# iebeid/ProtGram-DirectGCN

Hardware: AMD Instinct MI355X
Metric: edges/sec propagated, DirectGCN fwd on 4-gram graph, 1/2/4/8 MI355X (higher is better)
Workload: dtype f32; 1 GPU; directgcn_fwd_B(20,4); graph=complete n-gram de Bruijn B(20,4), num_nodes=160000, transitions=3200000, nnz_per_adjacency=6559580, feat_dim=128, layers=2, classes=20, propagation=precomputed-weights, entry=trainer COO (edge_index_*/edge_weight_* -> csr_from_coo), parallelism=single

## Files before the change

### include/pg_directgcn.h

```cpp
#ifndef PG_DIRECTGCN_H
#define PG_DIRECTGCN_H

#include <stdint.h>

#ifdef __cplusplus
extern "C" {
#endif

#define PG_ABI_VERSION 4

#define PG_OK 0
#define PG_ERR_ARG (-1)
#define PG_ERR_HIP (-2)
#define PG_ERR_UNSUPPORTED (-3)

typedef struct pg_edge3 {
    int32_t col;
    float w_in;
    float w_out;
    float w_und;
} pg_edge3_t;

typedef struct pg_edgeraw {
    int32_t col;
    float a_fwd;
    float a_bwd;
    float m_und;
} pg_edgeraw_t;

typedef struct pg_edge1 {
    int32_t col;
    float w;
} pg_edge1_t;


#define PG_FLAG_NO_XCD_REMAP (1u << 0)
#define PG_FLAG_EDGE_LDS (1u << 1)
#define PG_FLAG_UNROLL4 (1u << 2)
#define PG_FLAG_BCAST_RECORDS (1u << 7)
#define PG_FLAG_NGRAMT_WIDE (1u << 8)
#define PG_FLAG_NGRAMT_HALVES (1u << 4)
#define PG_FLAG_NGRAMT_NARROW (1u << 3)
#define PG_FLAG_DENSE_PREGATED (1u << 14)
#define PG_FLAG_DENSE_TILED (1u << 15)
#define PG_FLAG_DENSE_X3 (1u << 16)
#define PG_FLAG_WGRAD_BF16_TILED (1u << 11)
#define PG_FLAG_DGRAD_BF16_TILED (1u << 10)
#define PG_FLAG_DGRAD_BF16_RESIDENT (1u << 9)
#define PG_FLAG_WGRAD_F32MFMA (1u << 18)
#define PG_FLAG_DGRAD_F32MFMA (1u << 17)
#define PG_FLAG_NO_NGRAM (1u << 20)
#define PG_FLAG_NGRAM_BLOCK4 (1u << 21)
#define PG_FLAG_MID_NO_PAIRS (1u << 22)
#define PG_FLAG_MID_LOADER_SYNC (1u << 19)
#define PG_FLAG_DENSE_NO_IL (1u << 13)
#define PG_FLAG_DENSE_A_CACHED (1u << 12)
#define PG_FLAG_SCATTER_CPW_SHIFT 24
#define PG_FLAG_MID_TRANSPOSED (1u << 23)


const char* pg_last_error(void);
int pg_abi_version(void);

int pg_spmm3_f32(int64_t n_rows, const int64_t* rowptr, const int32_t* row_order, const pg_edge3_t* edges,
                 const float* X, int64_t ldx, int64_t F,
                 float* Z, int64_t ldz, uint32_t flags, void* stream);


int pg_spmm3_fusednorm_f32(int64_t n_rows, const int64_t* rowptr, const int32_t* row_order,
                           const pg_edgeraw_t* edges,
                           const float* node_norm, float eps,
                           const float* X, int64_t ldx, int64_t F,
                           float* Z, int64_t ldz, uint32_t flags, void* stream);

int pg_edges_normalize_f32(int64_t n_rows, const int64_t* rowptr, const pg_edgeraw_t* raw,
                           const float* node_norm, float eps, pg_edge3_t* out, void* stream);

int pg_spmm3t_f32(int64_t n_rows, const int64_t* rowptr, const int32_t* row_order, const pg_edge3_t* edges,
                  const float* G, int64_t ldg, int64_t F,
                  float* dX, int64_t lddx, int accumulate, uint32_t flags, void* stream);

int pg_spmm1_f32(int64_t n_rows, const int64_t* rowptr, const int32_t* row_order, const pg_edge1_t* edges,
                 const float* X, int64_t ldx, int64_t F,
                 float* Y, int64_t ldy, int accumulate, uint32_t flags, void* stream);

#define PG_GATES_VECTOR 0
#define PG_GATES_SCALAR 1

typedef struct pg_layer_args {
    int64_t M, F_in, F_out;
    const float* Z; int64_t ldz;
    const float* W_main_in; const float* W_main_out; const float* W_undirected; const float* W_shared;
    const float* b_main_in; const float* b_dir_shared_in;
    const float* b_main_out; const float* b_dir_shared_out;
    const float* b_undirected; const float* b_undirected_shared;
    int32_t gate_mode;
    const float* C_in; const float* C_out; const float* C_directed; const float* C_undirected; const float* C_all;
    const int64_t* rows;
    const float* constant; int64_t ld_const;
    const float* res_x; int64_t ld_res;
    const float* W_res; const float* b_res;
    int32_t act; float slope;
    float* Y; int64_t ldy;
    float drop_p; const int64_t* drop_seed;
} pg_layer_args_t;

int64_t pg_directgcn_packed_floats(int64_t F_in, int64_t F_out, int has_res_proj);

int pg_directgcn_pack_f32(const pg_layer_args_t* args, float* packed, void* stream);

int pg_directgcn_dense_f32(const pg_layer_args_t* args, const float* packed, uint32_t flags, void* stream);

int pg_directgcn_dense_ngram_rows_f32(const pg_layer_args_t* args, const float* packed, int64_t Kn1, int64_t m0,
                                      int32_t map_res, int32_t map_y, uint32_t flags, void* stream);

int pg_spmm3_gated_f32(int64_t n_rows, const int64_t* rowptr, const int32_t* row_order, const pg_edge3_t* edges,
                       const float* X, int64_t ldx, int64_t F, const pg_layer_args_t* gates,
                       float* Z, int64_t ldz, uint32_t flags, void* stream);

int64_t pg_ngram_plan_floats(int K, int n, int64_t n_rows);
int pg_ngram_plan_f32(int K, int n, int64_t n_rows, const int64_t* rowptr, const pg_edge3_t* edges, float* plan,
                      int64_t plan_floats, int* bad, void* stream);
int pg_spmm3_ngram_f32(int K, int n, int64_t n_rows, const float* plan, const float* X, int64_t ldx, int64_t F,
                       const pg_layer_args_t* gates, float* Z, int64_t ldz, uint32_t flags, void* stream);
int pg_spmm3t_ngram_f32(int K, int n, int64_t n_rows, const float* plan, const float* G, int64_t ldg, int64_t F,
                        float* dX, int64_t lddx, int accumulate, uint32_t flags, void* stream);
int pg_spmm3t_ngram_bf16(int K, int n, int64_t n_rows, const float* plan, const uint16_t* G, int64_t ldg, int64_t F,
                         uint16_t* dX, int64_t lddx, int accumulate, uint32_t flags, void* stream);
int pg_spmm3t_ngram_add_bf16(int K, int n, int64_t n_rows, const float* plan, const uint16_t* G, int64_t ldg,
                             int64_t F, const uint16_t* C, int64_t ldc, uint16_t* dX, int64_t lddx, uint32_t flags,
                             void* stream);

int64_t pg_ngram_mplan_floats(int K, int n, int64_t n_rows);
int pg_ngram_mplan_f32(int K, int n, int64_t n_rows, const int64_t* rowptr, const pg_edge3_t* edges, float* plan,
                       int64_t plan_floats, int* bad, void* stream);
int pg_spmm3_ngram_mid_f32(int K, int n, int64_t n_rows, const float* plan, const float* X, int64_t ldx, int64_t F,
                           const pg_layer_args_t* gates, float* Z, int64_t ldz, uint32_t flags, void* stream);
int pg_spmm3_ngram_mid_rows_f32(int K, int n, int64_t n_rows, const float* plan, const float* X, int64_t ldx, int64_t F,
                                int64_t m_begin, int64_t m_end, float* Z, int64_t ldz, uint32_t flags, void* stream);
// ... 144 lines not shown
```

### protgram-directgcn_amd/_lib.py

```python
from __future__ import annotations

import ctypes
import os

_HERE = os.path.dirname(os.path.abspath(__file__))
_LIB_PATH = os.environ.get("PG_DIRECTGCN_LIB", os.path.join(_HERE, "libpgdgcn.so"))

PG_OK = 0
PG_FLAG_NO_XCD_REMAP = 1 << 0
PG_FLAG_EDGE_LDS = 1 << 1
PG_FLAG_UNROLL4 = 1 << 2
PG_FLAG_BCAST_RECORDS = 1 << 7
PG_FLAG_NGRAMT_WIDE = 1 << 8
PG_FLAG_NGRAMT_NARROW = 1 << 3
PG_FLAG_NGRAMT_HALVES = 1 << 4
PG_FLAG_DENSE_PREGATED = 1 << 14
PG_FLAG_DENSE_TILED = 1 << 15
PG_FLAG_DENSE_X3 = 1 << 16
PG_FLAG_WGRAD_F32MFMA = 1 << 18
PG_FLAG_WGRAD_BF16_TILED = 1 << 11
PG_FLAG_DGRAD_BF16_TILED = 1 << 10
PG_FLAG_DGRAD_BF16_RESIDENT = 1 << 9
PG_FLAG_DGRAD_F32MFMA = 1 << 17
PG_FLAG_NO_NGRAM = 1 << 20
PG_FLAG_NGRAM_BLOCK4 = 1 << 21
PG_FLAG_MID_NO_PAIRS = 1 << 22
PG_FLAG_MID_LOADER_SYNC = 1 << 19
PG_FLAG_MID_TRANSPOSED = 1 << 23
PG_FLAG_SCATTER_CPW_SHIFT = 24
PG_FLAG_DENSE_A_CACHED = 1 << 12
PG_FLAG_DENSE_NO_IL = 1 << 13

c_i64, c_i32, c_u32, c_f32, c_vp = ctypes.c_int64, ctypes.c_int32, ctypes.c_uint32, ctypes.c_float, ctypes.c_void_p


PG_OK, PG_ERR_ARG, PG_ERR_HIP, PG_ERR_UNSUPPORTED = 0, -1, -2, -3


class NativeLibraryError(RuntimeError):
    pass


class LayerArgs(ctypes.Structure):
    _fields_ = [("M", c_i64), ("F_in", c_i64), ("F_out", c_i64),
                ("Z", c_vp), ("ldz", c_i64),
                ("W_main_in", c_vp), ("W_main_out", c_vp), ("W_undirected", c_vp), ("W_shared", c_vp),
                ("b_main_in", c_vp), ("b_dir_shared_in", c_vp),
                ("b_main_out", c_vp), ("b_dir_shared_out", c_vp),
                ("b_undirected", c_vp), ("b_undirected_shared", c_vp),
                ("gate_mode", c_i32),
                ("C_in", c_vp), ("C_out", c_vp), ("C_directed", c_vp), ("C_undirected", c_vp), ("C_all", c_vp),
                ("rows", c_vp),
                ("constant", c_vp), ("ld_const", c_i64),
                ("res_x", c_vp), ("ld_res", c_i64),
                ("W_res", c_vp), ("b_res", c_vp),
                ("act", c_i32), ("slope", c_f32),
                ("Y", c_vp), ("ldy", c_i64),
                ("drop_p", c_f32), ("drop_seed", c_vp)]


class LayerGradArgs(ctypes.Structure):
    _fields_ = [("dY", c_vp), ("lddy", c_i64), ("dpre", c_vp), ("ldp", c_i64), ("dZ", c_vp), ("lddz", c_i64),
                ("dres", c_vp), ("lddres", c_i64), ("dgate", c_vp), ("gates", c_vp), ("dW", c_vp),
                ("work", c_vp), ("work_floats", c_i64), ("dpre_f32", c_vp), ("ldp_f32", c_i64)]


SIGNATURES = {
    "pg_last_error": (ctypes.c_char_p, []),
    "pg_abi_version": (ctypes.c_int, []),
    "pg_spmm3_f32": (ctypes.c_int, [c_i64, c_vp, c_vp, c_vp, c_vp, c_i64, c_i64, c_vp, c_i64, c_u32, c_vp]),
    "pg_spmm3_gated_f32": (ctypes.c_int, [c_i64, c_vp, c_vp, c_vp, c_vp, c_i64, c_i64, ctypes.POINTER(LayerArgs), c_vp,
                                          c_i64, c_u32, c_vp]),
    "pg_spmm3_fusednorm_f32": (ctypes.c_int, [c_i64, c_vp, c_vp, c_vp, c_vp, c_f32, c_vp, c_i64, c_i64, c_vp, c_i64,
                                              c_u32, c_vp]),
    "pg_edges_normalize_f32": (ctypes.c_int, [c_i64, c_vp, c_vp, c_vp, c_f32, c_vp, c_vp]),
    "pg_ngram_plan_floats": (c_i64, [ctypes.c_int, ctypes.c_int, c_i64]),
    "pg_ngram_plan_f32": (ctypes.c_int, [ctypes.c_int, ctypes.c_int, c_i64, c_vp, c_vp, c_vp, c_i64, c_vp, c_vp]),
    "pg_spmm3_ngram_f32": (ctypes.c_int, [ctypes.c_int, ctypes.c_int, c_i64, c_vp, c_vp, c_i64, c_i64,
                                          ctypes.POINTER(LayerArgs), c_vp, c_i64, c_u32, c_vp]),
    "pg_ngram_mplan_floats": (c_i64, [ctypes.c_int, ctypes.c_int, c_i64]),
    "pg_ngram_mplan_f32": (ctypes.c_int, [ctypes.c_int, ctypes.c_int, c_i64, c_vp, c_vp, c_vp, c_i64, c_vp, c_vp]),
    "pg_spmm3_ngram_mid_f32": (ctypes.c_int, [ctypes.c_int, ctypes.c_int, c_i64, c_vp, c_vp, c_i64, c_i64,
                                              ctypes.POINTER(LayerArgs), c_vp, c_i64, c_u32, c_vp]),
    "pg_spmm3_ngram_mid_rows_f32": (ctypes.c_int, [ctypes.c_int, ctypes.c_int, c_i64, c_vp, c_vp, c_i64, c_i64, c_i64,
                                                   c_i64, c_vp, c_i64, c_u32, c_vp]),
    "pg_spmm3_ngram_mid_bf16": (ctypes.c_int, [ctypes.c_int, ctypes.c_int, c_i64, c_vp, c_vp, c_i64, c_i64, c_vp,
                                               c_i64, c_u32, c_vp]),
    "pg_spmm3_ngram_mid_rows_bf16": (ctypes.c_int, [ctypes.c_int, ctypes.c_int, c_i64, c_vp, c_vp, c_i64, c_i64, c_i64,
                                                    c_i64, c_vp, c_i64, c_u32, c_vp]),
    "pg_ngram_mplan_map_f32": (ctypes.c_int, [ctypes.c_int, ctypes.c_int, c_i64, c_vp, c_vp, c_vp, c_vp, c_i64, c_vp,
                                              c_vp]),
    "pg_spmm3_ngram_mid_map_f32": (ctypes.c_int, [ctypes.c_int, ctypes.c_int, c_vp, c_vp, c_vp, c_i64, c_i64, c_vp,
                                                  c_i64, c_u32, c_vp]),
    "pg_spmm3_resid_f32": (ctypes.c_int, [c_i64, c_vp, c_vp, c_vp, c_vp, c_i64, c_i64, c_vp, c_i64, c_u32, c_vp]),
    "pg_rows_gather": (ctypes.c_int, [c_vp, c_i64, c_vp, c_i64, c_i64, c_vp, c_i64, c_vp]),
    "pg_rows_scatter": (ctypes.c_int, [c_vp, c_i64, c_vp, c_i64, c_i64, c_vp, c_i64, c_vp]),
    "pg_rows_gather_sum": (ctypes.c_int, [c_vp, c_i64, c_vp, c_i64, ctypes.c_int, c_vp, c_vp, c_i64, c_i64, c_vp,
                                          c_i64, ctypes.c_int, c_vp]),
    "pg_ngram_scatter_plan": (ctypes.c_int, [ctypes.c_int, ctypes.c_int, c_vp, c_i64, c_i64, c_vp, c_vp]),
    "pg_spmm3t_ngram_scatter_f32": (ctypes.c_int, [c_vp, c_i64, c_vp, c_i64, c_i64, c_vp, c_i64, c_u32, c_vp]),
    "pg_spmm3t_ngram_scatter_bf16": (ctypes.c_int, [c_vp, c_i64, c_vp, c_i64, c_i64, c_vp, c_i64, c_u32, c_vp]),
    "pg_spmm3t_ngram_f32": (ctypes.c_int, [ctypes.c_int, ctypes.c_int, c_i64, c_vp, c_vp, c_i64, c_i64, c_vp, c_i64,
                                           ctypes.c_int, c_u32, c_vp]),
    "pg_spmm3t_ngram_mid_offdiag_f32": (ctypes.c_int, [ctypes.c_int, ctypes.c_int, c_i64, c_vp, c_vp, c_i64, c_i64,
                                                       c_vp, c_i64, ctypes.c_int, c_u32, c_vp]),
    "pg_spmm3t_ngram_mid_bf16": (ctypes.c_int, [ctypes.c_int, ctypes.c_int, c_i64, c_vp, c_vp, c_i64, c_i64, c_vp, c_i64,
                                                ctypes.c_int, c_u32, c_vp]),
    "pg_spmm3t_ngram_bf16": (ctypes.c_int, [ctypes.c_int, ctypes.c_int, c_i64, c_vp, c_vp, c_i64, c_i64, c_vp, c_i64,
                                            ctypes.c_int, c_u32, c_vp]),
    "pg_spmm3t_ngram_add_bf16": (ctypes.c_int, [ctypes.c_int, ctypes.c_int, c_i64, c_vp, c_vp, c_i64, c_i64, c_vp,
                                                c_i64, c_vp, c_i64, c_u32, c_vp]),
    "pg_spmm3t_f32": (ctypes.c_int, [c_i64, c_vp, c_vp, c_vp, c_vp, c_i64, c_i64, c_vp, c_i64, ctypes.c_int, c_u32,
                                     c_vp]),
    "pg_spmm1_f32": (ctypes.c_int, [c_i64, c_vp, c_vp, c_vp, c_vp, c_i64, c_i64, c_vp, c_i64, ctypes.c_int, c_u32,
# ... 82 lines not shown
```

### protgram-directgcn_amd/csrc/pg_dense.hip

```cpp
#include "pg_common.h"
#include "pg_split3.h"

namespace {

typedef float f32x16 __attribute__((ext_vector_type(16)));
typedef float f32x4 __attribute__((ext_vector_type(4)));

constexpr int BK = 32;
constexpr int LDSW = 36;

struct DenseP {
    int64_t M;
    int F_in, F_out, K;
    const float* Z;
    int64_t ldz;
    const float* Bp;
    const float* bsum;
    int gate_mode;
    const float *C_in, *C_out, *C_dir, *C_und, *C_all;
    const int64_t* rows;
    const float* constant;
    int64_t ld_const;
    const float* res_x;
    int64_t ld_res;
// ... 560 lines not shown
        const int64_t m0 = (lo + kt * step) * BMW;
        if (prev_full) asm volatile("s_waitcnt vmcnt(2)" ::: "memory");
        else asm volatile("s_waitcnt vmcnt(0)" ::: "memory");
        lds_barrier();
        issue_CR(tile_of(kt));
        if (wave == 0) issue_G(tile_of(kt + 1), buf ^ 1);
        convert(Af, buf);
        lds_barrier();
        issue_A(tile_of(kt + 1), Af);
        f32x4 acc[2] = {f32x4{0.f, 0.f, 0.f, 0.f}, f32x4{0.f, 0.f, 0.f, 0.f}};
        const uint4* ab0 = &As[0][a_unit(0, lc, kg)];
        const uint4* ab2 = &As[2][a_unit(0, lc, kg)];
        uint4 op[2][6];
        auto ld_ops = [&](int s, uint4 (&o)[6]) {
            o[0] = ab0[128 * s];
            o[1] = ab0[BMW * NU + 128 * s];
            o[2] = ab2[128 * s];
            o[3] = ab0[64 + 128 * s];
            o[4] = ab0[BMW * NU + 64 + 128 * s];
            o[5] = ab2[64 + 128 * s];
        };
        ld_ops(0, op[0]);
#pragma unroll
        for (int s = 0; s < NS; ++s) {
            if (s + 1 < NS) ld_ops(s + 1, op[(s + 1) & 1]);
            const uint4 a00 = op[s & 1][0], a01 = op[s & 1][1], a02 = op[s & 1][2];
            const uint4 a10 = op[s & 1][3], a11 = op[s & 1][4], a12 = op[s & 1][5];
            acc[0] = mfma_bf(a02, w0[s], acc[0]);
            acc[1] = mfma_bf(a12, w0[s], acc[1]);
            acc[0] = mfma_bf(a01, w1[s], acc[0]);
            acc[1] = mfma_bf(a11, w1[s], acc[1]);
            acc[0] = mfma_bf(a00, w2[s], acc[0]);
            acc[1] = mfma_bf(a10, w2[s], acc[1]);
            acc[0] = mfma_bf(a01, w0[s], acc[0]);
            acc[1] = mfma_bf(a11, w0[s], acc[1]);
            acc[0] = mfma_bf(a00, w1[s], acc[0]);
            acc[1] = mfma_bf(a10, w1[s], acc[1]);
            acc[0] = mfma_bf(a00, w0[s], acc[0]);
            acc[1] = mfma_bf(a10, w0[s], acc[1]);
            __builtin_amdgcn_sched_barrier(0);
        }
        lds_barrier();
#pragma unroll
        for (int sb = 0; sb < 2; ++sb)
#pragma unroll
            for (int i = 0; i < 4; ++i) lds_stf(&Es[(16 * sb + 4 * kg + i) * ELD + col], acc[sb][i]);
        if (wave == 0) asm volatile("s_waitcnt vmcnt(%0)" ::"n"(WAIT_W0) : "memory");
        else asm volatile("s_waitcnt vmcnt(%0)" ::"n"(WAIT_WN) : "memory");
        lds_barrier();
#pragma unroll
        for (int h = 0; h < 2; ++h) {
            const int rl = er + 16 * h;
            if (m0 + rl >= p.M) continue;
            float4 v, cv, rv, bb[4];
            lds_ld4x2(&Cs[rl * 128 + 4 * ej], &Rs[rl * 128 + 4 * ej], cv, rv);
            lds_ld4x4(&Es[rl * ELD + 4 * ej], &Bs[0][4 * ej], &Bs[1][4 * ej], &Bs[2][4 * ej], bb);
            v = bb[0];
            const float4 b0 = bb[1], b1 = bb[2], b2 = bb[3];
            float4 br;
            lds_ld4x2(&Bs[3][4 * ej], &Bs[3][4 * ej], br, br);
            if (!has_const) cv = make_float4(0.f, 0.f, 0.f, 0.f);
            if (!id_res) rv = make_float4(0.f, 0.f, 0.f, 0.f);
            float s0, s1, s2;
            gates(buf, rl, s0, s1, s2);
            const float o[4] = {v.x, v.y, v.z, v.w}, C4[4] = {cv.x, cv.y, cv.z, cv.w}, R4[4] = {rv.x, rv.y, rv.z, rv.w};
            const float B0[4] = {b0.x, b0.y, b0.z, b0.w}, B1[4] = {b1.x, b1.y, b1.z, b1.w},
                        B2[4] = {b2.x, b2.y, b2.z, b2.w}, BR[4] = {br.x, br.y, br.z, br.w};
            float y[4];
#pragma unroll
            for (int e = 0; e < 4; ++e) {
                const float qv = epi_sum(o[e], s0, s1, s2, B0[e], B1[e], B2[e], BR[e], C4[e], R4[e]);
                y[e] = (p.act && !(qv > 0.f)) ? qv * p.slope : qv;
                if (p.drop_s != 0.f) y[e] = drop_apply(p, dseed, m0 + rl, 4 * ej + e, y[e]);
            }
            *reinterpret_cast<float4*>(p.Y + (m0 + rl) * p.ldy + 4 * ej) = make_float4(y[0], y[1], y[2], y[3]);
        }
        prev_full = m0 + BMW <= p.M;
    }
    asm volatile("s_waitcnt vmcnt(0)" ::: "memory");
}

__device__ __forceinline__ int a_unit16(int s, int r, int g) { return 64 * s + 4 * r + (g ^ ((-(r >> 2)) & 3)); }

template <bool PRE, bool IL, bool DROP>
__global__ __launch_bounds__(512) void dense_x3p_kernel(DenseP p) {
    constexpr int F_IN = 128, K = 384;
    constexpr int CH = K / 4;
    constexpr int NU = K / 8;
    constexpr int NS = K / 32;
    constexpr int BM = 16;
    constexpr int NI = BM * CH / 64 / 8;
    constexpr int NG = 2;
    constexpr int NCR = 2;
    (void)NCR;
    constexpr int ELD = 128 + 4;
    static_assert(BM * CH % 512 == 0 && NI == 3, "tile shape");
    __shared__ __attribute__((aligned(16))) float Af0[BM * K];
    __shared__ __attribute__((aligned(16))) float Af1[BM * K];
    __shared__ __attribute__((aligned(16))) uint4 As[2][3][BM * NU];
    __shared__ __attribute__((aligned(16))) float Cs[BM * 128];
    __shared__ __attribute__((aligned(16))) float Rs[BM * 128];
    __shared__ __attribute__((aligned(16))) float Es[BM * ELD];
    __shared__ __attribute__((aligned(16))) float Gi[4][8][BM];
    __shared__ __attribute__((aligned(16))) float Bs[4][128];

    const int tid = threadIdx.x;
    const int wave = tid >> 6, lane = tid & 63;
    const int lc = lane & 15, kg = lane >> 4;
    const int col = 16 * wave + lc;
    const bool mfma_first = wave < 4;
    const uint64_t dseed = DROP ? drop_seed_of(p) : 0ull;
    const int64_t T = (p.M + BM - 1) / BM;
    DSTAMP_INIT;
    {
        const int q = tid >> 7, n = tid & 127;
        float bv = 0.f;
        if (p.rawW) {
            if (q < 3) bv = q == 0 ? p.bm0[n] + p.bs0[n] : q == 1 ? p.bm1[n] + p.bs1[n] : p.bm2[n] + p.bs2[n];
        } else if (q < 3 || p.proj_res) {
            bv = p.bsum[q * p.F_out + n];
        }
        Bs[q][n] = bv;
    }
    const int nb = gridDim.x, b = blockIdx.x;
    int64_t ntl, lo, step;
    if ((nb & 7) == 0 && nb >= 8) {
        const int x = b & 7, i = b >> 3, bpx = nb >> 3;
        const int64_t xlo = T * x / 8, xhi = T * (x + 1) / 8;
        ntl = (xhi - xlo - i + bpx - 1) / bpx;
        lo = xlo + i;
        step = bpx;
    } else {
        ntl = (T - b + nb - 1) / nb;
        lo = b;
        step = nb;
    }
    if (ntl < 0) ntl = 0;

    uint4 w0[NS], w1[NS], w2[NS];
    if (p.rawW) {
#pragma unroll
        for (int s = 0; s < NS; ++s) {
            const float* wq = s < 4 ? p.Wq0 : s < 8 ? p.Wq1 : p.Wq2;
            const int64_t o = (int64_t)col * F_IN + (32 * s) % F_IN + 4 * kg;
            const float4 a0 = ld4(wq + o), a1 = ld4(wq + o + 16), h0 = ld4(p.Wsh + o), h1 = ld4(p.Wsh + o + 16);
            const float v[8] = {a0.x + h0.x, a0.y + h0.y, a0.z + h0.z, a0.w + h0.w,
                                a1.x + h1.x, a1.y + h1.y, a1.z + h1.z, a1.w + h1.w};
            split8(v, w0[s], w1[s], w2[s]);
        }
    } else {
        const float* src = p.Bp + (int64_t)col * K + 4 * kg;
#pragma unroll
        for (int s = 0; s < NS; ++s) {
            const float4 x0 = ld4(src + 32 * s), x1 = ld4(src + 32 * s + 16);
            const float v[8] = {x0.x, x0.y, x0.z, x0.w, x1.x, x1.y, x1.z, x1.w};
            split8(v, w0[s], w1[s], w2[s]);
        }
    }
    const int ej = tid & 31, er = tid >> 5;
    const bool has_const = p.constant && p.gate_mode == PG_GATES_VECTOR;
    const bool id_res = p.res_x && !p.proj_res;
    auto tile_of = [&](int64_t kt) { return lo + max((int64_t)0, min(kt, ntl - 1)) * step; };

    auto issue_A_piece = [&](int64_t tile, float* Ad, int i) {
        if (DEXP(3)) return;
        const int64_t m0 = tile * BM;
        const int rmax = (int)min((int64_t)(BM - 1), p.M - 1 - m0);
        const float* zb = p.Z + m0 * p.ldz;
        int ln = lane;
        asm volatile("" : "+v"(ln));
        const int idx = (wave * NI + i) * 64 + ln;
        const int r = idx / CH, pos = idx - r * CH;
        const int k = 4 * (pos ^ r);
        const int rr = min(r, rmax);
        if (p.nt_a) glds16nt(zb + (rr * (int)p.ldz + k), Ad + (wave * NI + i) * 256);
        else glds16(zb + (rr * (int)p.ldz + k), Ad + (wave * NI + i) * 256);
    };
    auto issue_A = [&](int64_t tile, float* Ad) {
#pragma unroll
        for (int i = 0; i < NI; ++i) issue_A_piece(tile, Ad, i);
    };
    auto issue_G = [&](int64_t tile, int slot) {
        int ln = lane;
        asm volatile("" : "+v"(ln));
        const int64_t r = p.gate_mode == PG_GATES_SCALAR ? 0 : min(tile * BM + (ln & 15), p.M - 1);
        const float* c0 = p.C_in;
        const float* c1 = p.C_out;
        const float* c2 = p.C_dir;
        const float* c3 = p.C_und;
        const float* c4 = p.C_all;
        asm volatile("" : "+s"(c0), "+s"(c1), "+s"(c2), "+s"(c3), "+s"(c4));
        const int q = ln >> 4;
        const float* cq = q == 0 ? c0 : q == 1 ? c1 : q == 2 ? c2 : c3;
        glds4(cq + r, &Gi[slot][0][0]);
        glds4(c4 + r, &Gi[slot][4][0]);
    };
    auto issue_CR = [&](int64_t tile) {
        if (DEXP(4)) return;
        const int64_t m0 = tile * BM;
        const int rmax = (int)min((int64_t)(BM - 1), p.M - 1 - m0);
        int ln = lane;
        asm volatile("" : "+v"(ln));
        const int rr = min(2 * wave + (ln >> 5), rmax);
        const float* cb = has_const ? p.constant + m0 * p.ld_const + (rr * (int)p.ld_const) : p.Z + m0 * p.ldz;
        const float* rb = !id_res    ? p.Z + m0 * p.ldz
                          : p.map_res ? p.res_x + ngram_row(p, m0 + rr) * p.ld_res
                                      : p.res_x + m0 * p.ld_res + (rr * (int)p.ld_res);
        if (p.nt_a) glds16nt(cb + 4 * (ln & 31), Cs + wave * 256);
        else glds16(cb + 4 * (ln & 31), Cs + wave * 256);
        glds16(rb + 4 * (ln & 31), Rs + wave * 256);
    };
    auto gates = [&](int slot, int r, float& s0, float& s1, float& s2) {
        float c[5];
        lds_gates5<BM * 4>(&Gi[slot][0][r], c);
        const float cad = c[4] * c[2];
        s0 = cad * c[0];
        s1 = cad * c[1];
        s2 = c[4] * c[3];
    };
    auto split_tile = [&](const float* Af, int ab, int gslot) {
        if (DEXP(1)) return;
        const int r = tid & 15;
        const bool two = tid + 512 < BM * NU;
        const int u0 = tid >> 4, u1 = u0 + 32;
        const int c00 = 8 * (u0 >> 2) + (u0 & 3), c10 = 8 * (u1 >> 2) + (u1 & 3);
        float4 x[4];
        if (two) lds_ld4x4(&Af[r * K + 4 * (c00 ^ r)], &Af[r * K + 4 * ((c00 + 4) ^ r)], &Af[r * K + 4 * (c10 ^ r)],
                           &Af[r * K + 4 * ((c10 + 4) ^ r)], x);
        else lds_ld4x2(&Af[r * K + 4 * (c00 ^ r)], &Af[r * K + 4 * ((c00 + 4) ^ r)], x[0], x[1]);
        float sg[3] = {1.f, 1.f, 1.f};
        if (!PRE) gates(gslot, r, sg[0], sg[1], sg[2]);
#pragma unroll
        for (int i = 0; i < 2; ++i) {
            if (i == 1 && !two) break;
            const int u = i ? u1 : u0;
            const int s = u >> 2, g = u & 3;
            const float4 a = x[2 * i], c = x[2 * i + 1];
            float v[8] = {a.x, a.y, a.z, a.w, c.x, c.y, c.z, c.w};
            if (!PRE) {
                const float sc = sg[(32 * s) / F_IN];
#pragma unroll
                for (int e = 0; e < 8; ++e) v[e] = __fmul_rn(v[e], sc);
            }
            uint4 s0, s1, s2;
            split8(v, s0, s1, s2);
            const int pos = a_unit16(s, r, g);
            lds_st16(&As[ab][0][pos], s0);
            lds_st16(&As[ab][1][pos], s1);
            lds_st16(&As[ab][2][pos], s2);
        }
    };
    f32x4 acc = {0.f, 0.f, 0.f, 0.f};
    auto mfma_tile = [&](int ab, int64_t a_tile, float* a_dst, int g_slot, bool issue) {
        const uint4* a0 = &As[ab][0][a_unit16(0, lc, kg)];
        const uint4* a1 = &As[ab][1][a_unit16(0, lc, kg)];
        const uint4* a2 = &As[ab][2][a_unit16(0, lc, kg)];
        uint4 op[2][3];
        acc = f32x4{0.f, 0.f, 0.f, 0.f};
        if (DEXP(0)) {
            if (IL && issue) {
                issue_A(a_tile, a_dst);
                if (wave == 0) issue_G(a_tile, g_slot);
            }
            return;
        }
        op[0][0] = a0[0];
        op[0][1] = a1[0];
        op[0][2] = a2[0];
#pragma unroll
        for (int s = 0; s < NS; ++s) {
            if (s + 1 < NS) {
                op[(s + 1) & 1][0] = a0[64 * (s + 1)];
                op[(s + 1) & 1][1] = a1[64 * (s + 1)];
                op[(s + 1) & 1][2] = a2[64 * (s + 1)];
            }
            const uint4 x0 = op[s & 1][0], x1 = op[s & 1][1], x2 = op[s & 1][2];
            acc = mfma_bf(x2, w0[s], acc);
            acc = mfma_bf(x1, w1[s], acc);
            acc = mfma_bf(x0, w2[s], acc);
            acc = mfma_bf(x1, w0[s], acc);
            acc = mfma_bf(x0, w1[s], acc);
            acc = mfma_bf(x0, w0[s], acc);
            if constexpr (IL) {
                if (issue && (s == 2 || s == 5 || s == 8)) issue_A_piece(a_tile, a_dst, s / 3);
                if (issue && s == 10 && wave == 0) issue_G(a_tile, g_slot);
            }
            __builtin_amdgcn_sched_barrier(0);
        }
    };

    if (ntl > 0) {
        issue_A(tile_of(0), Af0);
        if (wave == 0) issue_G(tile_of(0), 0);
        issue_A(tile_of(1), Af1);
        if (wave == 0) issue_G(tile_of(1), 1);
        if (wave == 0) asm volatile("s_waitcnt vmcnt(%0)" ::"n"(NI + NG) : "memory");
        else asm volatile("s_waitcnt vmcnt(%0)" ::"n"(NI) : "memory");
        lds_barrier();
        split_tile(Af0, 0, 0);
    }
    float4 bq[4];
    if (ntl > 0) lds_ld4x4(&Bs[0][4 * ej], &Bs[1][4 * ej], &Bs[2][4 * ej], &Bs[3][4 * ej], bq);
    bool y_pending = false;
    for (int64_t i = 0; i <= ntl && ntl > 0; ++i) {
        const int ab = (int)(i & 1);
        [[maybe_unused]] const int si = (int)i;
        DSTAMP(si, 0);
        if (y_pending) asm volatile("s_waitcnt vmcnt(1)" ::: "memory");
        else asm volatile("s_waitcnt vmcnt(0)" ::: "memory");
        lds_barrier();
        DSTAMP(si, 1);
        if (i >= 1) {
#pragma unroll
            for (int e = 0; e < 4; ++e) lds_stf(&Es[(4 * kg + e) * ELD + col], acc[e]);
        }
        issue_CR(tile_of(i - 1));
        const int64_t a_tile = tile_of(i + 2);
        float* const a_dst = ab ? Af1 : Af0;
        const int g_slot = (int)((i + 2) & 3);
        const bool do_mfma = i < ntl, do_split = i + 1 < ntl;
        if (!IL || !do_mfma) {
            issue_A(a_tile, a_dst);
            if (wave == 0) issue_G(a_tile, g_slot);
        }
        DSTAMP(si, 2);
        if (mfma_first) {
            if (do_mfma) mfma_tile(ab, a_tile, a_dst, g_slot, IL);
            DSTAMP(si, 3);
            if (do_split) split_tile(ab ? Af0 : Af1, ab ^ 1, (int)((i + 1) & 3));
        } else {
            if (do_split) split_tile(ab ? Af0 : Af1, ab ^ 1, (int)((i + 1) & 3));
            DSTAMP(si, 3);
            if (do_mfma) mfma_tile(ab, a_tile, a_dst, g_slot, IL);
        }
        DSTAMP(si, 4);
        if (wave == 0) asm volatile("s_waitcnt vmcnt(%0)" ::"n"(NI + NG) : "memory");
        else asm volatile("s_waitcnt vmcnt(%0)" ::"n"(NI) : "memory");
        DSTAMP(si, 5);
        lds_barrier();
        DSTAMP(si, 6);
        y_pending = false;
        if (i >= 1) {
            const int64_t m0 = tile_of(i - 1) * BM;
            const int gs = (int)((i - 1) & 3);
            if (m0 + er < p.M) {
                float4 cv, rv, ov;
                float c[5];
                lds_epi<BM * 4>(&Cs[er * 128 + 4 * ej], &Rs[er * 128 + 4 * ej], &Es[er * ELD + 4 * ej], &Gi[gs][0][er],
                                cv, rv, ov, c);
                if (!has_const) cv = make_float4(0.f, 0.f, 0.f, 0.f);
                if (!id_res) rv = make_float4(0.f, 0.f, 0.f, 0.f);
                const float cad = c[4] * c[2];
                const float s0 = cad * c[0], s1 = cad * c[1], s2 = c[4] * c[3];
                const float o[4] = {ov.x, ov.y, ov.z, ov.w}, C4[4] = {cv.x, cv.y, cv.z, cv.w},
                            R4[4] = {rv.x, rv.y, rv.z, rv.w};
                const float B0[4] = {bq[0].x, bq[0].y, bq[0].z, bq[0].w}, B1[4] = {bq[1].x, bq[1].y, bq[1].z, bq[1].w},
                            B2[4] = {bq[2].x, bq[2].y, bq[2].z, bq[2].w}, BR[4] = {bq[3].x, bq[3].y, bq[3].z, bq[3].w};
                float y[4];
#pragma unroll
                for (int e = 0; e < 4; ++e) {
                    const float qv = epi_sum(o[e], s0, s1, s2, B0[e], B1[e], B2[e], BR[e], C4[e], R4[e]);
                    y[e] = (p.act && !(qv > 0.f)) ? qv * p.slope : qv;
                    if (DROP) y[e] = drop_apply(p, dseed, m0 + er, 4 * ej + e, y[e]);
                }
                if (!DEXP(2)) {
                    const int64_t yr = p.map_y ? ngram_row(p, m0 + er) : m0 + er;
                    *reinterpret_cast<float4*>(p.Y + yr * p.ldy + 4 * ej) = make_float4(y[0], y[1], y[2], y[3]);
                    y_pending = true;
                }
            }
        }
        DSTAMP(si, 7);
    }
    asm volatile("s_waitcnt vmcnt(0)" ::: "memory");
}

__global__ __launch_bounds__(256) void pack_kernel(int F_in, int F_out, int K, const float* W0, const float* W1,
                                                   const float* W2, const float* Ws, const float* Wr,
                                                   const float* bm0, const float* bs0, const float* bm1,
                                                   const float* bs1, const float* bm2, const float* bs2,
                                                   const float* br, float* out) {
    const int64_t total = (int64_t)F_out * K;
    for (int64_t i = (int64_t)blockIdx.x * 256 + threadIdx.x; i < total + 4 * F_out; i += (int64_t)gridDim.x * 256) {
        if (i < total) {
            const int n = (int)(i / K), k = (int)(i % K);
            const int q = seg_of(k, F_in), kk = k - q * F_in;
            const int64_t w = (int64_t)n * F_in + kk;
            float v;
            if (q == 0) v = W0[w] + Ws[w];
            else if (q == 1) v = W1[w] + Ws[w];
            else if (q == 2) v = W2[w] + Ws[w];
            else v = Wr[w];
            out[i] = v;
        } else {
            const int j = (int)(i - total), q = j / F_out, n = j % F_out;
            float v;
            if (q == 0) v = bm0[n] + bs0[n];
            else if (q == 1) v = bm1[n] + bs1[n];
            else if (q == 2) v = bm2[n] + bs2[n];
            else v = br ? br[n] : 0.f;
            out[i] = v;
        }
    }
}

}

extern "C" {

int64_t pg_directgcn_packed_floats(int64_t F_in, int64_t F_out, int has_res_proj) {
    return F_out * (has_res_proj ? 4 : 3) * F_in + 4 * F_out;
}

int pg_directgcn_pack_f32(const pg_layer_args_t* a, float* packed, void* stream) {
    PG_REQUIRE(a != nullptr && packed != nullptr, "null args");
    PG_REQUIRE(a->F_in > 0 && a->F_out > 0 && a->F_in < (1 << 20) && a->F_out < (1 << 20), "bad F_in/F_out");
    PG_REQUIRE(a->W_main_in && a->W_main_out && a->W_undirected && a->W_shared, "null weight");
    PG_REQUIRE(a->b_main_in && a->b_dir_shared_in && a->b_main_out && a->b_dir_shared_out && a->b_undirected &&
                   a->b_undirected_shared,
               "null bias");
    const int K = (int)((a->W_res ? 4 : 3) * a->F_in);
    const int64_t total = a->F_out * K + 4 * a->F_out;
    const int64_t nb = (total + 255) / 256 < 1024 ? (total + 255) / 256 : 1024;
    hipLaunchKernelGGL(pack_kernel, dim3((unsigned)nb), dim3(256), 0, (hipStream_t)stream, (int)a->F_in,
                       (int)a->F_out, K, a->W_main_in, a->W_main_out, a->W_undirected, a->W_shared, a->W_res,
                       a->b_main_in, a->b_dir_shared_in, a->b_main_out, a->b_dir_shared_out, a->b_undirected,
                       a->b_undirected_shared, a->b_res, packed);
    return pg::check_launch("pg_directgcn_pack_f32");
}

static int dense_launch(const pg_layer_args_t* a, const float* packed, uint32_t flags, const int64_t* ngmap,
                        void* stream) {
    PG_REQUIRE(a != nullptr, "null args");
    PG_REQUIRE(a->M >= 0 && a->F_in > 0 && a->F_out > 0 && a->F_in < (1 << 20) && a->F_out < (1 << 20),
               "bad shape M=%lld F_in=%lld F_out=%lld", (long long)a->M, (long long)a->F_in, (long long)a->F_out);
    if (a->M == 0) return PG_OK;
    PG_REQUIRE(a->Z && a->ldz >= 3 * a->F_in, "Z must be [M, >=3*F_in]");
    PG_REQUIRE(a->C_in && a->C_out && a->C_directed && a->C_undirected && a->C_all, "null gate");
    PG_REQUIRE(a->gate_mode == PG_GATES_VECTOR || a->gate_mode == PG_GATES_SCALAR, "bad gate_mode");
    PG_REQUIRE(!a->constant || a->ld_const >= a->F_out, "ld_const < F_out");
    PG_REQUIRE(!a->W_res || a->res_x, "W_res needs res_x");
    PG_REQUIRE(!a->res_x || a->W_res || a->F_in == a->F_out, "identity residual needs F_in == F_out");
    PG_REQUIRE(!a->res_x || a->ld_res >= a->F_in, "ld_res < F_in");
    PG_REQUIRE(a->Y && a->ldy >= a->F_out, "bad output");
    DenseP p{};
    p.M = a->M;
    p.F_in = (int)a->F_in;
    p.F_out = (int)a->F_out;
    p.K = (int)((a->W_res ? 4 : 3) * a->F_in);
    p.Z = a->Z;
    p.ldz = a->ldz;
    p.Bp = packed;
    p.bsum = packed ? packed + (int64_t)p.F_out * p.K : nullptr;
    if (!packed) {
        PG_REQUIRE(a->W_main_in && a->W_main_out && a->W_undirected && a->W_shared && a->b_main_in &&
                       a->b_dir_shared_in && a->b_main_out && a->b_dir_shared_out && a->b_undirected &&
                       a->b_undirected_shared,
                   "packed == NULL needs the raw weights and biases in the args");
        p.rawW = 1;
        p.Wq0 = a->W_main_in;
        p.Wq1 = a->W_main_out;
        p.Wq2 = a->W_undirected;
        p.Wsh = a->W_shared;
        p.bm0 = a->b_main_in;
        p.bs0 = a->b_dir_shared_in;
        p.bm1 = a->b_main_out;
        p.bs1 = a->b_dir_shared_out;
        p.bm2 = a->b_undirected;
        p.bs2 = a->b_undirected_shared;
    }
    p.gate_mode = a->gate_mode;
    p.C_in = a->C_in;
    p.C_out = a->C_out;
    p.C_dir = a->C_directed;
    p.C_und = a->C_undirected;
    p.C_all = a->C_all;
    p.rows = a->rows;
    p.constant = a->constant;
    p.ld_const = a->ld_const;
    p.res_x = a->res_x;
    p.ld_res = a->ld_res;
    p.proj_res = a->W_res ? 1 : 0;
    p.act = a->act;
    p.slope = a->slope;
    p.Y = a->Y;
    p.ldy = a->ldy;
    p.remap = (flags & PG_FLAG_NO_XCD_REMAP) ? 0 : 1;
    p.pregated = (flags & PG_FLAG_DENSE_PREGATED) ? 1 : 0;
    p.nt_a = (flags & PG_FLAG_DENSE_A_CACHED) ? 0 : 1;
    if (const int rc = pg::drop_params(a, p.drop_thr, p.drop_s)) return rc;
    p.drop_seed = a->drop_seed;
    PG_REQUIRE(p.drop_s == 0.f || a->M * a->F_out <= (int64_t(1) << 32), "fused dropout: M * F_out > 2^32");
#ifdef PG_DENSE_EXP
    p.exp = (int)((flags >> 24) & 31u);
#endif
    if (ngmap) {
        p.map_kn1 = ngmap[0];
        p.map_m0 = ngmap[1];
        p.map_res = ngmap[2] ? 1 : 0;
        p.map_y = ngmap[3] ? 1 : 0;
    }
    p.vec_out = (a->F_out % 4 == 0) && (a->ldy % 4 == 0) && pg::aligned16(a->Y) &&
                (!a->constant || (a->ld_const % 4 == 0 && pg::aligned16(a->constant))) &&
                (!a->res_x || a->W_res || (a->ld_res % 4 == 0 && pg::aligned16(a->res_x)));
    bool vec = (a->F_in % 4 == 0) && (a->ldz % 4 == 0) && pg::aligned16(a->Z) && pg::aligned16(packed);
    if (a->res_x) vec = vec && pg::aligned16(a->res_x) && (a->ld_res % 4 == 0);
    const bool wide = a->F_out > 64;
    const int64_t BN = wide ? 128 : 64;
    const int64_t nb = ((a->M + 127) / 128) * ((a->F_out + BN - 1) / BN);
    hipStream_t s = (hipStream_t)stream;
    const bool ws_shape_ok = a->F_out == 128 && vec && p.vec_out &&
                             (!a->res_x || (a->ld_res % 4 == 0 && pg::aligned16(a->res_x)));
    if (!(flags & PG_FLAG_DENSE_TILED) && ws_shape_ok && a->ldz < (1 << 24) && a->rows == nullptr &&
        (!a->res_x || a->ld_res < (1 << 24)) &&
        ((a->F_in == 128 && !a->W_res) || (a->F_in == 64 && a->W_res))) {
        if (ngmap && a->F_in != 128)
            return pg::set_error(PG_ERR_UNSUPPORTED, "pg_directgcn_dense_ngram_rows_f32: F_in = F_out = 128 only");
        int dev = 0, ncu = 256;
        if (hipGetDevice(&dev) != hipSuccess ||
            hipDeviceGetAttribute(&ncu, hipDeviceAttributeMultiprocessorCount, dev) != hipSuccess || ncu <= 0)
            ncu = 256;
        if (a->F_in == 128) {
            if (p.rawW && !(pg::aligned16(a->W_main_in) && pg::aligned16(a->W_main_out) &&
                            pg::aligned16(a->W_undirected) && pg::aligned16(a->W_shared)))
                return pg::set_error(PG_ERR_UNSUPPORTED, "pg_directgcn_dense_f32: unpacked weights must be 16-B aligned");
            const int64_t T16 = (a->M + 15) / 16;
            const unsigned g16 = (unsigned)(T16 < ncu ? T16 : ncu);
            const bool il = (flags & PG_FLAG_DENSE_NO_IL) == 0;
            if (p.drop_s != 0.f) {
                if (p.pregated) hipLaunchKernelGGL((dense_x3p_kernel<true, true, true>), dim3(g16), dim3(512), 0, s, p);
                else hipLaunchKernelGGL((dense_x3p_kernel<false, true, true>), dim3(g16), dim3(512), 0, s, p);
            } else if (p.pregated) {
                if (il) hipLaunchKernelGGL((dense_x3p_kernel<true, true, false>), dim3(g16), dim3(512), 0, s, p);
                else hipLaunchKernelGGL((dense_x3p_kernel<true, false, false>), dim3(g16), dim3(512), 0, s, p);
            } else {
                if (il) hipLaunchKernelGGL((dense_x3p_kernel<false, true, false>), dim3(g16), dim3(512), 0, s, p);
                else hipLaunchKernelGGL((dense_x3p_kernel<false, false, false>), dim3(g16), dim3(512), 0, s, p);
            }
        } else {
            if (p.rawW)
                return pg::set_error(PG_ERR_UNSUPPORTED, "pg_directgcn_dense_f32: unpacked weights need the pipelined "
                                                         "split-bf16 kernel (F_in = F_out = 128, no row map)");
            const int64_t T = (a->M + 31) / 32;
            const unsigned g = (unsigned)(T < ncu ? T : ncu);
            if (p.pregated) hipLaunchKernelGGL((dense_x3_kernel<64, 4, true>), dim3(g), dim3(512), 0, s, p);
            else hipLaunchKernelGGL((dense_x3_kernel<64, 4, false>), dim3(g), dim3(512), 0, s, p);
        }
        return pg::check_launch("pg_directgcn_dense_f32");
    }
    if (ngmap)
        return pg::set_error(PG_ERR_UNSUPPORTED, "pg_directgcn_dense_ngram_rows_f32: needs the pipelined split-bf16 "
                                                 "kernel's shape (F_in = F_out = 128, no W_res, no row map, aligned)");
    if (p.rawW)
        return pg::set_error(PG_ERR_UNSUPPORTED, "pg_directgcn_dense_f32: unpacked weights need the pipelined "
                                                 "split-bf16 kernel (F_in = F_out = 128, no row map)");
    if (vec) {
        if (wide) hipLaunchKernelGGL((dense_kernel<128, 128, 8, true>), dim3((unsigned)nb), dim3(512), 0, s, p);
        else hipLaunchKernelGGL((dense_kernel<128, 64, 8, true>), dim3((unsigned)nb), dim3(512), 0, s, p);
    } else {
        if (wide) hipLaunchKernelGGL((dense_kernel<128, 128, 8, false>), dim3((unsigned)nb), dim3(512), 0, s, p);
        else hipLaunchKernelGGL((dense_kernel<128, 64, 8, false>), dim3((unsigned)nb), dim3(512), 0, s, p);
    }
    return pg::check_launch("pg_directgcn_dense_f32");
}

int pg_directgcn_dense_f32(const pg_layer_args_t* a, const float* packed, uint32_t flags, void* stream) {
    return dense_launch(a, packed, flags, nullptr, stream);
}

#ifdef PG_DENSE_EXP
int pg_dense_set_stamps(unsigned long long* buf) {
    return hipMemcpyToSymbol(HIP_SYMBOL(g_dense_stamps), &buf, sizeof(buf)) == hipSuccess ? PG_OK : PG_ERR_HIP;
}
#endif

int pg_directgcn_dense_ngram_rows_f32(const pg_layer_args_t* a, const float* packed, int64_t Kn1, int64_t m0,
                                      int32_t map_res, int32_t map_y, uint32_t flags, void* stream) {
    PG_REQUIRE(a != nullptr, "null args");
    int64_t pw = 20;
    while (pw < Kn1 && pw <= (int64_t(1) << 56)) pw *= 20;
    PG_REQUIRE(Kn1 >= 20 && pw == Kn1 && m0 >= 0 && m0 < Kn1,
               "bad n-gram map (Kn1 = %lld must be a power of K = 20; m0 = %lld)", (long long)Kn1, (long long)m0);
    PG_REQUIRE(a->M % 400 == 0 && a->M < (int64_t(1) << 31), "rows must be whole middles (M = %lld)", (long long)a->M);
    PG_REQUIRE(!map_res || a->res_x, "map_res needs res_x");
    PG_REQUIRE(m0 + a->M / 400 <= Kn1 / 20, "middles [%lld, %lld) past the graph's %lld", (long long)m0,
               (long long)(m0 + a->M / 400), (long long)(Kn1 / 20));
    const int64_t map[4] = {Kn1, m0, map_res, map_y};
    return dense_launch(a, packed, flags, map, stream);
}

}
```

Before: 78.01 billion edges/s.

## Apply dense epilogue directly from MFMA registers instead of staging through LDS

Adds a new default path in the pipelined split-bf16 dense kernel. The MFMA operand order is swapped so each lane holds a row-contiguous 4-column slice of the output, and the epilogue runs straight from the accumulator registers on the same tile. The constant and residual rows are loaded into registers before the MFMAs rather than staged through LDS. This drops the Cs/Rs/Es shared buffers, one barrier-synchronised LDS round trip and the one-tile epilogue lag. The old LDS-staged epilogue stays available behind a new flag; the trade-off is more live registers and less latency hiding for the output stores.

```diff
diff --git a/include/pg_directgcn.h b/include/pg_directgcn.h
--- a/include/pg_directgcn.h
+++ b/include/pg_directgcn.h
@@ -55,6 +55,7 @@
 #define PG_FLAG_MID_LOADER_SYNC (1u << 19)
 #define PG_FLAG_DENSE_NO_IL (1u << 13)
 #define PG_FLAG_DENSE_A_CACHED (1u << 12)
+#define PG_FLAG_DENSE_LDS_EPILOGUE (1u << 29)
 #define PG_FLAG_SCATTER_CPW_SHIFT 24
 #define PG_FLAG_MID_TRANSPOSED (1u << 23)
 
diff --git a/protgram-directgcn_amd/_lib.py b/protgram-directgcn_amd/_lib.py
--- a/protgram-directgcn_amd/_lib.py
+++ b/protgram-directgcn_amd/_lib.py
@@ -30,6 +30,7 @@
 PG_FLAG_SCATTER_CPW_SHIFT = 24
 PG_FLAG_DENSE_A_CACHED = 1 << 12
 PG_FLAG_DENSE_NO_IL = 1 << 13
+PG_FLAG_DENSE_LDS_EPILOGUE = 1 << 29
 
 c_i64, c_i32, c_u32, c_f32, c_vp = ctypes.c_int64, ctypes.c_int32, ctypes.c_uint32, ctypes.c_float, ctypes.c_void_p
 
diff --git a/protgram-directgcn_amd/csrc/pg_dense.hip b/protgram-directgcn_amd/csrc/pg_dense.hip
--- a/protgram-directgcn_amd/csrc/pg_dense.hip
+++ b/protgram-directgcn_amd/csrc/pg_dense.hip
@@ -666,7 +666,7 @@
 
 __device__ __forceinline__ int a_unit16(int s, int r, int g) { return 64 * s + 4 * r + (g ^ ((-(r >> 2)) & 3)); }
 
-template <bool PRE, bool IL, bool DROP>
+template <bool PRE, bool IL, bool DROP, bool LDSE>
 __global__ __launch_bounds__(512) void dense_x3p_kernel(DenseP p) {
     constexpr int F_IN = 128, K = 384;
     constexpr int CH = K / 4;
@@ -677,14 +677,14 @@
     constexpr int NG = 2;
     constexpr int NCR = 2;
     (void)NCR;
-    constexpr int ELD = 128 + 4;
+    [[maybe_unused]] constexpr int ELD = 128 + 4;
     static_assert(BM * CH % 512 == 0 && NI == 3, "tile shape");
     __shared__ __attribute__((aligned(16))) float Af0[BM * K];
     __shared__ __attribute__((aligned(16))) float Af1[BM * K];
     __shared__ __attribute__((aligned(16))) uint4 As[2][3][BM * NU];
-    __shared__ __attribute__((aligned(16))) float Cs[BM * 128];
-    __shared__ __attribute__((aligned(16))) float Rs[BM * 128];
-    __shared__ __attribute__((aligned(16))) float Es[BM * ELD];
+    __shared__ __attribute__((aligned(16))) float Cs[LDSE ? BM * 128 : 4];
+    __shared__ __attribute__((aligned(16))) float Rs[LDSE ? BM * 128 : 4];
+    __shared__ __attribute__((aligned(16))) float Es[LDSE ? BM * ELD : 4];
     __shared__ __attribute__((aligned(16))) float Gi[4][8][BM];
     __shared__ __attribute__((aligned(16))) float Bs[4][128];
 
@@ -741,7 +741,7 @@
             split8(v, w0[s], w1[s], w2[s]);
         }
     }
-    const int ej = tid & 31, er = tid >> 5;
+    const int ec = LDSE ? 4 * (tid & 31) : 16 * wave + 4 * kg, er = LDSE ? tid >> 5 : lc;
     const bool has_const = p.constant && p.gate_mode == PG_GATES_VECTOR;
     const bool id_res = p.res_x && !p.proj_res;
     auto tile_of = [&](int64_t kt) { return lo + max((int64_t)0, min(kt, ntl - 1)) * step; };
@@ -779,7 +779,32 @@
         glds4(cq + r, &Gi[slot][0][0]);
         glds4(c4 + r, &Gi[slot][4][0]);
     };
-    auto issue_CR = [&](int64_t tile) {
+    [[maybe_unused]] f32x4 cv = {0.f, 0.f, 0.f, 0.f}, rv = cv;
+    [[maybe_unused]] auto load_CR = [&](int64_t tile) {
+        if (DEXP(4)) return;
+        const int64_t m0 = tile * BM;
+        const int rmax = (int)min((int64_t)(BM - 1), p.M - 1 - m0);
+        const int rr = min(er, rmax);
+        const float* cb = has_const ? p.constant + m0 * p.ld_const + (rr * (int)p.ld_const) : p.Z + m0 * p.ldz;
+        const float* rb = !id_res    ? p.Z + m0 * p.ldz
+                          : p.map_res ? p.res_x + ngram_row(p, m0 + rr) * p.ld_res
+                                      : p.res_x + m0 * p.ld_res + (rr * (int)p.ld_res);
+        if (p.nt_a)
+            asm volatile("global_load_dwordx4 %0, %2, off nt\n\tglobal_load_dwordx4 %1, %3, off"
+                         : "=&v"(cv), "=&v"(rv)
+                         : "v"(cb + ec), "v"(rb + ec)
+                         : "memory");
+        else
+            asm volatile("global_load_dwordx4 %0, %2, off\n\tglobal_load_dwordx4 %1, %3, off"
+                         : "=&v"(cv), "=&v"(rv)
+                         : "v"(cb + ec), "v"(rb + ec)
+                         : "memory");
+    };
+    [[maybe_unused]] auto wait_CR = [&]() {
+        if (wave == 0) asm volatile("s_waitcnt vmcnt(%2)" : "+v"(cv), "+v"(rv) : "n"(NI + NG) : "memory");
+        else asm volatile("s_waitcnt vmcnt(%2)" : "+v"(cv), "+v"(rv) : "n"(NI) : "memory");
+    };
+    [[maybe_unused]] auto issue_CR = [&](int64_t tile) {
         if (DEXP(4)) return;
         const int64_t m0 = tile * BM;
         const int rmax = (int)min((int64_t)(BM - 1), p.M - 1 - m0);
@@ -859,12 +884,21 @@
                 op[(s + 1) & 1][2] = a2[64 * (s + 1)];
             }
             const uint4 x0 = op[s & 1][0], x1 = op[s & 1][1], x2 = op[s & 1][2];
-            acc = mfma_bf(x2, w0[s], acc);
-            acc = mfma_bf(x1, w1[s], acc);
-            acc = mfma_bf(x0, w2[s], acc);
-            acc = mfma_bf(x1, w0[s], acc);
-            acc = mfma_bf(x0, w1[s], acc);
-            acc = mfma_bf(x0, w0[s], acc);
+            if constexpr (LDSE) {
+                acc = mfma_bf(x2, w0[s], acc);
+                acc = mfma_bf(x1, w1[s], acc);
+                acc = mfma_bf(x0, w2[s], acc);
+                acc = mfma_bf(x1, w0[s], acc);
+                acc = mfma_bf(x0, w1[s], acc);
+                acc = mfma_bf(x0, w0[s], acc);
+            } else {
+                acc = mfma_bf(w0[s], x2, acc);
+                acc = mfma_bf(w1[s], x1, acc);
+                acc = mfma_bf(w2[s], x0, acc);
+                acc = mfma_bf(w0[s], x1, acc);
+                acc = mfma_bf(w1[s], x0, acc);
+                acc = mfma_bf(w0[s], x0, acc);
+            }
             if constexpr (IL) {
                 if (issue && (s == 2 || s == 5 || s == 8)) issue_A_piece(a_tile, a_dst, s / 3);
                 if (issue && s == 10 && wave == 0) issue_G(a_tile, g_slot);
@@ -884,77 +918,126 @@
         split_tile(Af0, 0, 0);
     }
     float4 bq[4];
-    if (ntl > 0) lds_ld4x4(&Bs[0][4 * ej], &Bs[1][4 * ej], &Bs[2][4 * ej], &Bs[3][4 * ej], bq);
-    bool y_pending = false;
-    for (int64_t i = 0; i <= ntl && ntl > 0; ++i) {
-        const int ab = (int)(i & 1);
-        [[maybe_unused]] const int si = (int)i;
-        DSTAMP(si, 0);
-        if (y_pending) asm volatile("s_waitcnt vmcnt(1)" ::: "memory");
-        else asm volatile("s_waitcnt vmcnt(0)" ::: "memory");
-        lds_barrier();
-        DSTAMP(si, 1);
-        if (i >= 1) {
-#pragma unroll
-            for (int e = 0; e < 4; ++e) lds_stf(&Es[(4 * kg + e) * ELD + col], acc[e]);
-        }
-        issue_CR(tile_of(i - 1));
-        const int64_t a_tile = tile_of(i + 2);
-        float* const a_dst = ab ? Af1 : Af0;
-        const int g_slot = (int)((i + 2) & 3);
-        const bool do_mfma = i < ntl, do_split = i + 1 < ntl;
-        if (!IL || !do_mfma) {
-            issue_A(a_tile, a_dst);
-            if (wave == 0) issue_G(a_tile, g_slot);
-        }
-        DSTAMP(si, 2);
-        if (mfma_first) {
-            if (do_mfma) mfma_tile(ab, a_tile, a_dst, g_slot, IL);
-            DSTAMP(si, 3);
-            if (do_split) split_tile(ab ? Af0 : Af1, ab ^ 1, (int)((i + 1) & 3));
-        } else {
-            if (do_split) split_tile(ab ? Af0 : Af1, ab ^ 1, (int)((i + 1) & 3));
-            DSTAMP(si, 3);
-            if (do_mfma) mfma_tile(ab, a_tile, a_dst, g_slot, IL);
-        }
-        DSTAMP(si, 4);
-        if (wave == 0) asm volatile("s_waitcnt vmcnt(%0)" ::"n"(NI + NG) : "memory");
-        else asm volatile("s_waitcnt vmcnt(%0)" ::"n"(NI) : "memory");
-        DSTAMP(si, 5);
-        lds_barrier();
-        DSTAMP(si, 6);
-        y_pending = false;
-        if (i >= 1) {
-            const int64_t m0 = tile_of(i - 1) * BM;
-            const int gs = (int)((i - 1) & 3);
-            if (m0 + er < p.M) {
-                float4 cv, rv, ov;
+    if (ntl > 0) lds_ld4x4(&Bs[0][ec], &Bs[1][ec], &Bs[2][ec], &Bs[3][ec], bq);
+    auto epilogue = [&](int64_t m0, float4 ov, float4 cq, float4 rq, const float (&c)[5]) {
+        if (!has_const) cq = make_float4(0.f, 0.f, 0.f, 0.f);
+        if (!id_res) rq = make_float4(0.f, 0.f, 0.f, 0.f);
+        const float cad = c[4] * c[2];
+        const float s0 = cad * c[0], s1 = cad * c[1], s2 = c[4] * c[3];
+        const float o[4] = {ov.x, ov.y, ov.z, ov.w}, C4[4] = {cq.x, cq.y, cq.z, cq.w}, R4[4] = {rq.x, rq.y, rq.z, rq.w};
+        const float B0[4] = {bq[0].x, bq[0].y, bq[0].z, bq[0].w}, B1[4] = {bq[1].x, bq[1].y, bq[1].z, bq[1].w},
+                    B2[4] = {bq[2].x, bq[2].y, bq[2].z, bq[2].w}, BR[4] = {bq[3].x, bq[3].y, bq[3].z, bq[3].w};
+        float y[4];
+#pragma unroll
+        for (int e = 0; e < 4; ++e) {
+            const float qv = epi_sum(o[e], s0, s1, s2, B0[e], B1[e], B2[e], BR[e], C4[e], R4[e]);
+            y[e] = (p.act && !(qv > 0.f)) ? qv * p.slope : qv;
+            if (DROP) y[e] = drop_apply(p, dseed, m0 + er, ec + e, y[e]);
+        }
+        const int64_t yr = p.map_y ? ngram_row(p, m0 + er) : m0 + er;
+        *reinterpret_cast<float4*>(p.Y + yr * p.ldy + ec) = make_float4(y[0], y[1], y[2], y[3]);
+    };
+    if constexpr (!LDSE) {
+        bool y_pending = false;
+        for (int64_t i = 0; i < ntl; ++i) {
+            const int ab = (int)(i & 1);
+            [[maybe_unused]] const int si = (int)i;
+            DSTAMP(si, 0);
+            if (y_pending) asm volatile("s_waitcnt vmcnt(1)" ::: "memory");
+            else asm volatile("s_waitcnt vmcnt(0)" ::: "memory");
+            lds_barrier();
+            DSTAMP(si, 1);
+            const int64_t m0 = tile_of(i) * BM;
+            load_CR(tile_of(i));
+            __builtin_amdgcn_sched_barrier(0);
+            const int64_t a_tile = tile_of(i + 2);
+            float* const a_dst = ab ? Af1 : Af0;
+            const int g_slot = (int)((i + 2) & 3);
+            const bool do_split = i + 1 < ntl;
+            if (!IL) {
+                issue_A(a_tile, a_dst);
+                if (wave == 0) issue_G(a_tile, g_slot);
+            }
+            DSTAMP(si, 2);
+            auto mfma_epi = [&](int pt) {
+                mfma_tile(ab, a_tile, a_dst, g_slot, IL);
+                DSTAMP(si, pt);
+                wait_CR();
+                DSTAMP(si, pt + 1);
                 float c[5];
-                lds_epi<BM * 4>(&Cs[er * 128 + 4 * ej], &Rs[er * 128 + 4 * ej], &Es[er * ELD + 4 * ej], &Gi[gs][0][er],
-                                cv, rv, ov, c);
-                if (!has_const) cv = make_float4(0.f, 0.f, 0.f, 0.f);
-                if (!id_res) rv = make_float4(0.f, 0.f, 0.f, 0.f);
-                const float cad = c[4] * c[2];
-                const float s0 = cad * c[0], s1 = cad * c[1], s2 = c[4] * c[3];
-                const float o[4] = {ov.x, ov.y, ov.z, ov.w}, C4[4] = {cv.x, cv.y, cv.z, cv.w},
-                            R4[4] = {rv.x, rv.y, rv.z, rv.w};
-                const float B0[4] = {bq[0].x, bq[0].y, bq[0].z, bq[0].w}, B1[4] = {bq[1].x, bq[1].y, bq[1].z, bq[1].w},
-                            B2[4] = {bq[2].x, bq[2].y, bq[2].z, bq[2].w}, BR[4] = {bq[3].x, bq[3].y, bq[3].z, bq[3].w};
-                float y[4];
-#pragma unroll
-                for (int e = 0; e < 4; ++e) {
-                    const float qv = epi_sum(o[e], s0, s1, s2, B0[e], B1[e], B2[e], BR[e], C4[e], R4[e]);
-                    y[e] = (p.act && !(qv > 0.f)) ? qv * p.slope : qv;
-                    if (DROP) y[e] = drop_apply(p, dseed, m0 + er, 4 * ej + e, y[e]);
+                lds_gates5<BM * 4>(&Gi[(int)(i & 3)][0][er], c);
+                if (!DEXP(2) && m0 + er < p.M) {
+                    epilogue(m0, make_float4(acc[0], acc[1], acc[2], acc[3]), make_float4(cv[0], cv[1], cv[2], cv[3]),
+                             make_float4(rv[0], rv[1], rv[2], rv[3]), c);
                 }
-                if (!DEXP(2)) {
-                    const int64_t yr = p.map_y ? ngram_row(p, m0 + er) : m0 + er;
-                    *reinterpret_cast<float4*>(p.Y + yr * p.ldy + 4 * ej) = make_float4(y[0], y[1], y[2], y[3]);
-                    y_pending = true;
+                DSTAMP(si, pt + 2);
+            };
+            if (mfma_first) {
+                mfma_epi(3);
+                if (do_split) split_tile(ab ? Af0 : Af1, ab ^ 1, (int)((i + 1) & 3));
+                DSTAMP(si, 6);
+            } else {
+                if (do_split) split_tile(ab ? Af0 : Af1, ab ^ 1, (int)((i + 1) & 3));
+                DSTAMP(si, 3);
+                mfma_epi(4);
+            }
+            y_pending = !DEXP(2) && m0 + BM <= p.M;
+        }
+    } else {
+        bool y_pending = false;
+        for (int64_t i = 0; i <= ntl && ntl > 0; ++i) {
+            const int ab = (int)(i & 1);
+            [[maybe_unused]] const int si = (int)i;
+            DSTAMP(si, 0);
+            if (y_pending) asm volatile("s_waitcnt vmcnt(1)" ::: "memory");
+            else asm volatile("s_waitcnt vmcnt(0)" ::: "memory");
+            lds_barrier();
+            DSTAMP(si, 1);
+            if (i >= 1) {
+#pragma unroll
+                for (int e = 0; e < 4; ++e) lds_stf(&Es[(4 * kg + e) * ELD + col], acc[e]);
+            }
+            issue_CR(tile_of(i - 1));
+            const int64_t a_tile = tile_of(i + 2);
+            float* const a_dst = ab ? Af1 : Af0;
+            const int g_slot = (int)((i + 2) & 3);
+            const bool do_mfma = i < ntl, do_split = i + 1 < ntl;
+            if (!IL || !do_mfma) {
+                issue_A(a_tile, a_dst);
+                if (wave == 0) issue_G(a_tile, g_slot);
+            }
+            DSTAMP(si, 2);
+            if (mfma_first) {
+                if (do_mfma) mfma_tile(ab, a_tile, a_dst, g_slot, IL);
+                DSTAMP(si, 3);
+                if (do_split) split_tile(ab ? Af0 : Af1, ab ^ 1, (int)((i + 1) & 3));
+            } else {
+                if (do_split) split_tile(ab ? Af0 : Af1, ab ^ 1, (int)((i + 1) & 3));
+                DSTAMP(si, 3);
+                if (do_mfma) mfma_tile(ab, a_tile, a_dst, g_slot, IL);
+            }
+            DSTAMP(si, 4);
+            if (wave == 0) asm volatile("s_waitcnt vmcnt(%0)" ::"n"(NI + NG) : "memory");
+            else asm volatile("s_waitcnt vmcnt(%0)" ::"n"(NI) : "memory");
+            DSTAMP(si, 5);
+            lds_barrier();
+            DSTAMP(si, 6);
+            y_pending = false;
+            if (i >= 1) {
+                const int64_t m0 = tile_of(i - 1) * BM;
+                const int gs = (int)((i - 1) & 3);
+                if (m0 + er < p.M) {
+                    float4 cq, rq, ov;
+                    float c[5];
+                    lds_epi<BM * 4>(&Cs[er * 128 + ec], &Rs[er * 128 + ec], &Es[er * ELD + ec], &Gi[gs][0][er], cq, rq, ov, c);
+                    if (!DEXP(2)) {
+                        epilogue(m0, ov, cq, rq, c);
+                        y_pending = true;
+                    }
                 }
             }
-        }
-        DSTAMP(si, 7);
+            DSTAMP(si, 7);
+        }
     }
     asm volatile("s_waitcnt vmcnt(0)" ::: "memory");
 }
@@ -1111,16 +1194,17 @@
             const int64_t T16 = (a->M + 15) / 16;
             const unsigned g16 = (unsigned)(T16 < ncu ? T16 : ncu);
             const bool il = (flags & PG_FLAG_DENSE_NO_IL) == 0;
-            if (p.drop_s != 0.f) {
-                if (p.pregated) hipLaunchKernelGGL((dense_x3p_kernel<true, true, true>), dim3(g16), dim3(512), 0, s, p);
-                else hipLaunchKernelGGL((dense_x3p_kernel<false, true, true>), dim3(g16), dim3(512), 0, s, p);
-            } else if (p.pregated) {
-                if (il) hipLaunchKernelGGL((dense_x3p_kernel<true, true, false>), dim3(g16), dim3(512), 0, s, p);
-                else hipLaunchKernelGGL((dense_x3p_kernel<true, false, false>), dim3(g16), dim3(512), 0, s, p);
-            } else {
-                if (il) hipLaunchKernelGGL((dense_x3p_kernel<false, true, false>), dim3(g16), dim3(512), 0, s, p);
-                else hipLaunchKernelGGL((dense_x3p_kernel<false, false, false>), dim3(g16), dim3(512), 0, s, p);
-            }
+            const bool ldse = (flags & PG_FLAG_DENSE_LDS_EPILOGUE) != 0;
+            const bool drop = p.drop_s != 0.f;
+            void (*kern)(DenseP);
+#define PG_X3P_PICK(LDSE)                                                                                  \
+    kern = drop ? (p.pregated ? dense_x3p_kernel<true, true, true, LDSE> : dense_x3p_kernel<false, true, true, LDSE>) \
+           : p.pregated ? (il ? dense_x3p_kernel<true, true, false, LDSE> : dense_x3p_kernel<true, false, false, LDSE>) \
+                        : (il ? dense_x3p_kernel<false, true, false, LDSE> : dense_x3p_kernel<false, false, false, LDSE>)
+            if (ldse) PG_X3P_PICK(true);
+            else PG_X3P_PICK(false);
+#undef PG_X3P_PICK
+            hipLaunchKernelGGL(kern, dim3(g16), dim3(512), 0, s, p);
         } else {
             if (p.rawW)
                 return pg::set_error(PG_ERR_UNSUPPORTED, "pg_directgcn_dense_f32: unpacked weights need the pipelined "
```

New measurement: 80.22 billion edges/s (median of 6 runs). 2.8% higher.
